# sencheng/CoBeL-RL

Measured on AMD Instinct MI355X. Metric: gridworld env-steps/sec (whole job), higher is better.
Workload: dtype f32

## Files before the change

cobel-rl_amd/csrc/tabular_pwg.hip:

```cpp
#include <stdlib.h>
#include <string.h>

#include "cobel_common.h"
#include "cobel_policy.h"

namespace {

constexpr int kHashBytes = 128 * 8;
constexpr int kMaxSlices = 8;
constexpr uint32_t kWholeTicket = 0x40000000u;
constexpr uint32_t kWholeThenSlices = 0x80000000u;
constexpr uint32_t kWholeSlice = 0xffu;
constexpr uint32_t kAbortWord = COBEL_TAB_SCRATCH_ABORT_WORD;
constexpr uint32_t kRingSpinLimit = 1u << 22;
struct pwg_args {
  const cobel_wrec* rec;
  const uint16_t* starts;
  const int32_t* start_off;
  int32_t S, n_worlds;
  cobel_tab_run_t r;
  uint64_t thr[16][3];
  float alpha_f, gamma_f, model_lr_f;
  int32_t nl, ng;
  uint32_t* queue;
  uint32_t reserve;
  int32_t n_slices;
  int32_t slice_steps[kMaxSlices];
  uint32_t whole;
  uint32_t* owner;
  uint32_t* tail;
  uint32_t* ring;
  uint32_t ring_stride;
  uint32_t xcc_limit;
};

#if defined(COBEL_PWG_NT)
#define NT_LD(p) __builtin_nontemporal_load(p)
#define NT_ST(v, p) __builtin_nontemporal_store(v, p)
#else
#define NT_LD(p) (*(p))
#define NT_ST(v, p) (*(p) = (v))
#endif

__device__ __forceinline__ void stores_done() { asm volatile("s_waitcnt vmcnt(0)" ::: "memory"); }

#if defined(COBEL_PWG_STAMPS)
__device__ __forceinline__ void pwg_stamp(uint32_t* stamps, uint32_t* prev, int k, int lane) {
  if (lane == 0) {
    const uint32_t now = (uint32_t)__builtin_readcyclecounter();
    atomicAdd(stamps + k, now - *prev);
    *prev = now;
  }
}
#define PWG_STAMP(k) pwg_stamp(stamps, stamp_prev, k, lane)
#else
#define PWG_STAMP(k)
#endif

typedef const __attribute__((address_space(4))) pwg_args* pwg_kargs;
__device__ __forceinline__ pwg_kargs rare_args() {
#if defined(__HIP_DEVICE_COMPILE__)
  pwg_kargs p = (pwg_kargs)__builtin_amdgcn_kernarg_segment_ptr();
  asm volatile("" : "+s"(p));
  return p;
#else
  return nullptr;
#endif
}

template <bool QG, bool POW2>
__device__ __forceinline__ void pwg_instance(const pwg_args& A, const int i, const int step_budget,
                                             unsigned char* const lds, const int lane,
                                             const uint64_t thr_mine, const uint32_t stripe
#if defined(COBEL_PWG_STAMPS)
                                             , uint32_t* stamps, uint32_t* stamp_prev
#endif
                                             ) {
  const int S = A.S;
  float4* const Qs = reinterpret_cast<float4*>(lds);
  float* const Qf = reinterpret_cast<float*>(lds);
  unsigned long long* const H = reinterpret_cast<unsigned long long*>(lds);
  const uint32_t g = A.r.instance_base + (uint32_t)i;
  const int world = (int)(g % (uint32_t)A.n_worlds);
  const uint4* const W4 = reinterpret_cast<const uint4*>(A.rec + (size_t)world * S);
  float4* const Qg = reinterpret_cast<float4*>(A.r.q) + (size_t)i * S;
  float* const Qgf = reinterpret_cast<float*>(Qg);
  uint64_t* const model = A.r.model + (size_t)i * S * 4;
  const uint32_t* const model32 = reinterpret_cast<const uint32_t*>(model);
  const uint32_t SA = (uint32_t)S * 4u;
  uint16_t* const Mg = A.r.model_index + (size_t)i * SA;
  uint32_t succ_sel = (lane & 2) ? 0xffffffffu : 0u, succ_sh = (uint32_t)(lane & 1) * 16u;
  uint32_t SAv = POW2 ? (uint32_t)__builtin_clz(SA) + 1u : SA;
  uint32_t qlane = (uint32_t)(lane & 3);
  asm volatile("" : "+v"(succ_sel), "+v"(succ_sh), "+v"(SAv), "+v"(qlane));
  auto succ_of = [&](uint32_t w0, uint32_t w1) -> uint32_t {
    return (((w1 & succ_sel) | (w0 & ~succ_sel)) >> succ_sh) & 0xffffu;
  };

  int32_t* const inst = A.r.inst + (size_t)i * COBEL_I_WORDS;
  int state = inst[COBEL_I_STATE];
  int step = inst[COBEL_I_STEP];
  int trial = inst[COBEL_I_TRIAL];
  uint32_t ce = (uint32_t)inst[COBEL_I_CTR_ENV];
  uint32_t cp = (uint32_t)inst[COBEL_I_CTR_POLICY];
  uint32_t cm = (uint32_t)inst[COBEL_I_CTR_MEMORY];
  uint32_t iflags = (uint32_t)inst[COBEL_I_FLAGS];
  double trew = *reinterpret_cast<const double*>(inst + COBEL_I_REWARD_LO + (lane & 0));
  asm volatile("" : "+v"(trew));
  uint32_t nonzero = 0u;
  if (QG) {
    for (int s0 = 0; s0 < S; s0 += 512) {
      float4 qv[8];
#pragma unroll
      for (int j = 0; j < 8; ++j) {
        const int s = s0 + j * 64 + lane;
        qv[j] = Qg[s < S ? s : S - 1];
      }
#pragma unroll
      for (int j = 0; j < 8; ++j)
        nonzero |= fbits(qv[j].x) | fbits(qv[j].y) | fbits(qv[j].z) | fbits(qv[j].w);
    }
  } else {
    for (int s0 = 0; s0 < S; s0 += 64) {
      const int s = s0 + lane;
      if (s < S)
        __builtin_amdgcn_global_load_lds(
            (const __attribute__((address_space(1))) void*)(Qg + s),
            (__attribute__((address_space(3))) void*)(Qs + s0), 16, 0, 0);
    }
  }

  const int B = A.r.batch;
#if defined(COBEL_PWG_SSEED)
  auto seed_now = [&]() -> uint64_t {
    uint64_t sd = A.r.seed;
    asm volatile("" : "+s"(sd));
    return sd;
  };
#else
  uint64_t seed_v = A.r.seed;
  asm volatile("" : "+v"(seed_v));
  auto seed_now = [&]() -> uint64_t { return seed_v; };
#endif
  double alpha = A.r.alpha, gamma = A.r.gamma;
  float alpha_f = A.alpha_f, gamma_f = A.gamma_f, mlr_f = A.model_lr_f;
  asm volatile("" : "+v"(alpha), "+v"(gamma), "+v"(alpha_f), "+v"(gamma_f), "+v"(mlr_f));

  uint32_t cw0 = 0, cw1 = 0;
  uint4 cand = {0, 0, 0, 0};
  cobel_u4 blk = {0, 0, 0, 0};
  int refresh_in = 0;
  uint2 mdig = {0u, 0u};
  uint32_t fix_sa = ~0u;
  float fix_r = 0.0f;
  uint32_t idx_cur = 0, mg_cur = 0;

  auto draw_m = [&](uint32_t counter) -> uint32_t {
    const cobel_u4 b = cobel_philox(counter >> 2, (uint32_t)lane, g, COBEL_STREAM_MEMORY, seed_now());
    return cobel_word(b, counter & 3u);
  };
  auto refresh_draws = [&](uint32_t pq) {
    const uint32_t mi = (cm + 1u) >> 2;
    const bool p0 = lane == 62, p1 = lane == 63;
    blk = cobel_philox(p1 ? 2u * pq + 1u : (p0 ? 2u * pq : mi), (p0 || p1) ? 0u : (uint32_t)lane,
                       g, (p0 || p1) ? COBEL_STREAM_POLICY : COBEL_STREAM_MEMORY, seed_now());
  };
  auto enter_state = [&](int s) {
    const uint4 c = W4[s];
    cw0 = rfl(c.x);
    cw1 = rfl(c.y);
    cand = W4[succ_of(cw0, cw1)];
    mdig = *reinterpret_cast<const uint2*>(&Mg[(uint32_t)s * 4u]);
  };
  auto begin_trial = [&]() -> bool {
    const pwg_kargs R = rare_args();
    if (trial >= R->r.trials_target) return false;
    const int start_lo = R->start_off[world];
    const uint32_t start_cnt = (uint32_t)(R->start_off[world + 1] - start_lo);
    state = (int)R->starts[start_lo + (int)cobel_draw_bounded(ce, 0u, g, COBEL_STREAM_ENV, seed_now(),
                                                              start_cnt)];
    ce += 1u;
    step = 0;
    trew = 0.0;
    asm volatile("" : "+v"(trew));
    iflags |= 1u;
    enter_state(state);
    return true;
  };
  auto plan_td = [&](float q, float m, float r, uint32_t nt) -> float {
    const double gnt = gamma * (double)nt;
    double td = (double)r + gnt * (double)m;
    td = td - (double)q;
    return (float)((double)q + alpha * td);
  };
  auto conflict_sets = [&](uint32_t idx, uint32_t ns) -> unsigned long long {
    unsigned long long* const H1 = H;
    unsigned long long* const H2 = H + 64;
    const uint32_t h1 = idx & 63u, h2 = idx >> 6;
    const unsigned long long bit = 1ull << lane;
    atomicOr(&H1[h1], bit);
    atomicOr(&H2[h2], bit);
    __builtin_amdgcn_wave_barrier();
    const ulonglong2* const r4 = reinterpret_cast<const ulonglong2*>(&H1[(ns & 15u) * 4u]);
    const ulonglong2 ra = r4[0], rb = r4[1];
    const unsigned long long cell = H1[h1] & H2[h2];
    const unsigned long long row = ((ra.x | ra.y) | (rb.x | rb.y)) & H2[ns >> 4];
    const unsigned long long cnd = (cell | row) & (bit - 1ull);
    __builtin_amdgcn_wave_barrier();
    H1[h1] = 0ull;
    H2[h2] = 0ull;
    return cnd;
  };
  uint32_t* const Qu = reinterpret_cast<uint32_t*>(lds);
  const uint4* const Qs4u = reinterpret_cast<const uint4*>(lds);
  uint32_t tag_mine = ~(uint32_t)lane;
  auto tag_round = [&](uint32_t idx, uint32_t ns, bool act, bool ch, float q, float qn, int lo) -> int {
    if (ch) atomicMax(&Qu[idx], tag_mine);
    __builtin_amdgcn_wave_barrier();
    uint32_t t = 0u, c2 = 0u;
    if (act) {
      const uint4 r2 = Qs4u[ns];
      c2 = Qu[idx];
      t = max(max(max(r2.x, r2.y), r2.z), max(r2.w, c2));
    }
    const unsigned long long blocked = __builtin_amdgcn_ballot_w64(act && t > tag_mine);
    const int stop = max(blocked ? __ffsll((long long)blocked) - 1 : B, lo + 1);
    if (ch && c2 == tag_mine) Qf[idx] = lane < stop ? qn : q;
    __builtin_amdgcn_wave_barrier();
    return stop;
  };
  auto run_batch_lds = [&](uint32_t idx, uint32_t ns, uint32_t nt, float r) {
    int first;
    {
      const float4 row = Qs[ns];
      const float q = Qf[idx];
      const float qn = plan_td(q, max4(row), r, nt);
      const bool ch = fbits(qn) != fbits(q);
      if (!__builtin_amdgcn_ballot_w64(ch)) return;
      first = tag_round(idx, ns, true, ch, q, qn, 0);
    }
    while (first < B) {
      const bool act = lane >= first;
      float q = 0.0f, qn = 0.0f;
      if (act) {
        const float4 row = Qs[ns];
        q = Qf[idx];
        qn = plan_td(q, max4(row), r, nt);
      }
      const bool ch = act && fbits(qn) != fbits(q);
      if (!__ballot(ch)) return;
      first = tag_round(idx, ns, act, ch, q, qn, first);
    }
  };
  auto run_batch_glb = [&](uint32_t idx, uint32_t ns, uint32_t nt, float r, float4 row, float q) {
    int first = B;
    bool have_conf = false;
    unsigned long long conf = 0ull;
    auto take_writes = [&](unsigned long long pend, float qn) {
      while (__ballot(pend != 0ull)) {
        const int e = pend ? (__ffsll((long long)pend) - 1) : 0;
        const uint32_t ie = (uint32_t)__shfl((int)idx, e);
        const float ve = __shfl(qn, e);
        if (pend) {
          if (ie == idx) q = ve;
          if ((ie >> 2) == ns) {
            const uint32_t c = ie & 3u;
            row.x = c == 0u ? ve : row.x;
            row.y = c == 1u ? ve : row.y;
            row.z = c == 2u ? ve : row.z;
            row.w = c == 3u ? ve : row.w;
          }
          pend &= pend - 1ull;
        }
      }
    };
    {
      const float qn = plan_td(q, max4(row), r, nt);
      const bool ch = fbits(qn) != fbits(q);
      const unsigned long long changed = __builtin_amdgcn_ballot_w64(ch);
      if (!changed) return;
      conf = conflict_sets(idx, ns);
      have_conf = true;
      const unsigned long long blocked = __builtin_amdgcn_ballot_w64((conf & changed) != 0ull);
      if (blocked) first = __ffsll((long long)blocked) - 1;
      if (ch && lane < first) Qgf[idx] = qn;
      if (first < B) {
        const unsigned long long committed = changed & ((1ull << first) - 1ull);
        take_writes(lane >= first ? (conf & committed) : 0ull, qn);
      }
    }
    while (first < B) {
      const bool act = lane >= first;
      float qn = q;
      if (act) qn = plan_td(q, max4(row), r, nt);
      const bool ch = act && fbits(qn) != fbits(q);
      const unsigned long long changed = __ballot(ch);
      int stop = B;
      if (changed) {
        if (!have_conf) {
          conf = conflict_sets(idx, ns);
          have_conf = true;
        }
        const unsigned long long blocked = __ballot(act && (conf & changed) != 0ull);
        if (blocked) stop = __ffsll((long long)blocked) - 1;
        if (ch && lane < stop) Qgf[idx] = qn;
        if (stop < B) {
          const unsigned long long committed = changed & ((1ull << stop) - 1ull);
          take_writes(lane >= stop ? (conf & committed) : 0ull, qn);
        }
      }
      first = stop;
    }
  };

  uint32_t warm;
  {
    const uint32_t off = (uint32_t)lane * 128u, last = SA * 2u - 4u;
    warm = *reinterpret_cast<const uint32_t*>(reinterpret_cast<const char*>(Mg) + (off < last ? off : last));
  }
  bool live = true;
  if (iflags & 1u) enter_state(state);
  else live = begin_trial();
  refresh_draws(cp >> 2);
  {
    const int jp = 3 - (int)(cp & 3u), jm = 4 - (int)((cm + 1u) & 3u);
    refresh_in = jp < jm ? jp : jm;
  }
  idx_cur = lane < B ? cobel_bounded(draw_m(cm), SA) : 0u;
  mg_cur = lane < B ? (uint32_t)Mg[idx_cur] : 0u;
  asm volatile("" ::"v"(warm));
  if (!QG) {
    stores_done();
    for (int s = lane; s < S; s += 64) {
      const float4 qv = Qs[s];
      nonzero |= fbits(qv.x) | fbits(qv.y) | fbits(qv.z) | fbits(qv.w);
    }
  }
  if (QG) {
    for (int b = lane; b < 128; b += 64) H[b] = 0ull;
    __builtin_amdgcn_wave_barrier();
  }
  if (!__ballot(nonzero != 0u)) {
    const uint2* const M2 = reinterpret_cast<const uint2*>(Mg);
    for (int s0 = 0; s0 < S; s0 += 512) {
      uint2 mv[8];
#pragma unroll
      for (int j = 0; j < 8; ++j) {
        const int s = s0 + j * 64 + lane;
        mv[j] = M2[s < S ? s : S - 1];
      }
#pragma unroll
      for (int j = 0; j < 8; ++j) nonzero |= (mv[j].x | mv[j].y) & 0x80008000u;
    }
  }
  if (__ballot(nonzero != 0u)) iflags |= 2u;

  PWG_STAMP(1);
  const int budget0 = step_budget > 0 ? step_budget : 0x7fffffff;
  int budget = budget0;
  uint32_t batches = 0u;
  asm volatile("" : "+v"(batches));

  while (live) {
    if (budget == 0) break;
    budget -= 1;

    const int src_lane = 62 + (int)((cp >> 1) & 1u);
    const uint32_t w0 = rl((cp & 1u) ? blk.z : blk.x, src_lane);
    const uint32_t w1 = rl((cp & 1u) ? blk.w : blk.y, src_lane);
    if (__builtin_expect(refresh_in == 0, 0)) {
      refresh_draws((cp + 1u) >> 2);
      const int jp = 4 - (int)((cp + 1u) & 3u), jm = 4 - (int)((cm + 1u) & 3u);
      refresh_in = jp < jm ? jp : jm;
    }
    refresh_in -= 1;
    cp += 1u;

    const uint32_t succ = succ_of(cw0, cw1);
    float4 srow;
    float qc;
    float4 prow = {0.0f, 0.0f, 0.0f, 0.0f};
    float pq = 0.0f;
    if (QG) {
      stores_done();
      qc = Qgf[(uint32_t)state * 4u + qlane];
      srow = Qg[succ];
      if (lane < B && (iflags & 2u)) {
        prow = Qg[mg_cur & 0x3fffu];
        pq = Qgf[idx_cur];
      }
    } else {
      qc = Qf[(uint32_t)state * 4u + qlane];
      srow = Qs[succ];
    }
    const float smax = max4(srow);

    int a;
    {
      float m;
      asm("s_nop 1\n\t"
          "v_max_f32_dpp %0, %1, %1 quad_perm:[1,0,3,2] row_mask:0xf bank_mask:0xf\n\t"
          "s_nop 1\n\t"
          "v_max_f32_dpp %0, %0, %0 quad_perm:[2,3,0,1] row_mask:0xf bank_mask:0xf"
          : "=&v"(m)
          : "v"(qc));
      const int t = (int)((uint32_t)__ballot(qc == m) & 15u);
      const uint64_t K = cobel_u53(w0, w1);
      const unsigned long long passed = __ballot(thr_mine <= K);
      a = __popcll((passed >> (t * 3)) & 7ull);
    }
    const int ns = (int)next_of(cw0, cw1, a);
    const uint32_t nw0 = rl(cand.x, a), nw1 = rl(cand.y, a);
    const uint32_t r_bits = rl(cand.z, a);
    const float r = __builtin_bit_cast(float, r_bits);
    if (r_bits != 0u) iflags |= 2u;
    const uint32_t end = rl(cand.w, a);
    const float ns_max = __builtin_bit_cast(float, rl(fbits(smax), a));
    const uint32_t nt = 1u - end;
    const uint32_t sa = (uint32_t)state * 4u + (uint32_t)a;
    const bool trial_over = end || (step + 1 >= A.r.steps_per_trial);
    const uint32_t dpair = rfl((a & 2) ? mdig.y : mdig.x);
    const uint32_t dold = (a & 1) ? (dpair >> 16) : (dpair & 0xffffu);
    float R = 0.0f;
    if (__builtin_expect((dold & 0x8000u) != 0u, 0)) {
      R = __builtin_bit_cast(float, rfl(model32[2u * sa]));
    }
    __builtin_amdgcn_sched_barrier(0);
    cand = W4[succ_of(nw0, nw1)];
    const uint2 mdig_next = *reinterpret_cast<const uint2*>(&Mg[(uint32_t)ns * 4u]);

    if (sa == fix_sa) R = fix_r;
    const float d = r - R;
    const float Rn = R + mlr_f * d;
    const uint32_t fresh_idx = sa;
    const float fresh_r = Rn;
    const uint32_t fresh_m = (uint32_t)ns | (nt << 14) | (fbits(Rn) ? 0x8000u : 0u);
    fix_sa = sa;
    fix_r = Rn;
    const float q_sa = __builtin_bit_cast(float, rl(fbits(qc), a));
    const float gnt = nt ? gamma_f : 0.0f;
    float td = r + gnt * ns_max;
    td = td - q_sa;
    const float qn_online = q_sa + alpha_f * td;
    if (lane == 0) {
      if (QG) Qgf[sa] = qn_online;
      else Qf[sa] = qn_online;
      NT_ST(cobel_model_pack(fresh_r, (uint32_t)ns, nt), &model[sa]);
      Mg[sa] = (uint16_t)fresh_m;
    }
    __builtin_amdgcn_wave_barrier();

    trew += (double)r;
    const int s_prev = state;
    state = ns;
    cw0 = nw0;
    cw1 = nw1;

    {
      uint32_t idx_next = 0u, mg_next = 0u;
      const uint32_t m = (idx_cur == fresh_idx) ? fresh_m : mg_cur;
      if (lane < B) {
        float rj = 0.0f;
        idx_next = POW2 ? cobel_word(blk, (cm + 1u) & 3u) >> SAv
                        : cobel_bounded(cobel_word(blk, (cm + 1u) & 3u), SAv);
        mg_next = (uint32_t)Mg[idx_next];
        if (iflags & 2u) {
          batches += 1u;
          if (__builtin_expect((m & 0x8000u) != 0u, 0)) {
            rj = __builtin_bit_cast(float, model32[2u * idx_cur]);
            asm volatile("" : "+v"(rj));
          }
          if (idx_cur == fresh_idx) rj = fresh_r;
          const uint32_t nsj = m & 0x3fffu;
          if (QG) {
            if (__ballot(idx_cur == fresh_idx)) {
              const float4 nrow = {__builtin_bit_cast(float, rl(fbits(srow.x), a)),
                                   __builtin_bit_cast(float, rl(fbits(srow.y), a)),
                                   __builtin_bit_cast(float, rl(fbits(srow.z), a)),
                                   __builtin_bit_cast(float, rl(fbits(srow.w), a))};
              if (idx_cur == fresh_idx) prow = nrow;
            }
            if (idx_cur == sa) pq = qn_online;
            if (nsj == (uint32_t)s_prev) {
              prow.x = a == 0 ? qn_online : prow.x;
              prow.y = a == 1 ? qn_online : prow.y;
              prow.z = a == 2 ? qn_online : prow.z;
              prow.w = a == 3 ? qn_online : prow.w;
            }
            run_batch_glb(idx_cur, nsj, (m >> 14) & 1u, rj, prow, pq);
          } else {
            run_batch_lds(idx_cur, nsj, (m >> 14) & 1u, rj);
          }
        }
        if (idx_next == fresh_idx) mg_next = fresh_m;
      }
      idx_cur = idx_next;
      mg_cur = mg_next;
      mdig = mdig_next;
      cm += 1u;
    }

    if (__builtin_expect(trial_over, 0)) {
      const pwg_kargs R = rare_args();
#define rr (R->r)
      if (lane == 0 && trial >= 0 && trial < rr.trial_cap) {
        const size_t mo = (size_t)stripe * (size_t)rr.trial_cap + (size_t)trial;
        if (rr.lat_sum) atomicAdd(rr.lat_sum + mo, (unsigned long long)step);
        if (rr.lat_cnt) atomicAdd(rr.lat_cnt + mo, 1ull);
        if (rr.reward_sum) atomicAdd(rr.reward_sum + mo, trew);
        if (rr.resp_cnt && trew > 0.0) atomicAdd(rr.resp_cnt + mo, 1ull);
        if (rr.lat_trace) rr.lat_trace[(size_t)i * rr.trial_cap + trial] = step;
      }
#undef rr
      trial += 1;
      iflags &= ~1u;
      if (!begin_trial()) break;
    } else {
      step += 1;
    }
  }

  __builtin_amdgcn_wave_barrier();
  PWG_STAMP(2);
  if (!QG) {
    for (int s0 = 0; s0 < S; s0 += 256) {
      float4 qv[4];
#pragma unroll
      for (int j = 0; j < 4; ++j) {
        const int s = s0 + j * 64 + lane;
        qv[j] = Qs[s < S ? s : S - 1];
      }
#pragma unroll
      for (int j = 0; j < 4; ++j) {
        const int s = s0 + j * 64 + lane;
        if (s < S) Qg[s] = qv[j];
      }
    }
  }
  if (lane == 0) {
    inst[COBEL_I_STATE] = state;
    inst[COBEL_I_STEP] = step;
    inst[COBEL_I_TRIAL] = trial;
    inst[COBEL_I_CTR_ENV] = (int32_t)ce;
    inst[COBEL_I_CTR_POLICY] = (int32_t)cp;
    inst[COBEL_I_CTR_MEMORY] = (int32_t)cm;
    inst[COBEL_I_FLAGS] = (int32_t)(iflags & ~2u);
    const unsigned long long executed = (unsigned long long)(budget0 - budget);
    *reinterpret_cast<double*>(inst + COBEL_I_REWARD_LO) = trew;
    *reinterpret_cast<unsigned long long*>(inst + COBEL_I_STEPS_LO) += executed;
    const pwg_kargs R = rare_args();
    if (R->r.steps_done && executed) atomicAdd(R->r.steps_done, executed);
    if (R->r.batches_done && batches) atomicAdd(R->r.batches_done, (unsigned long long)batches);
  }
  __builtin_amdgcn_wave_barrier();
}

template <bool SLICED, bool POW2>
__global__ __launch_bounds__(1024) void k_tab_pwg(const pwg_args A) {
  extern __shared__ __attribute__((aligned(16))) unsigned char lds_raw[];
  const int lane = (int)(threadIdx.x & 63u);
  const int wave = (int)rfl(threadIdx.x >> 6);
  const int waves = A.nl + A.ng;
  const size_t slice_l = (size_t)A.S * 16;
  const bool qg = wave >= A.nl;
  unsigned char* const lds =
      lds_raw + (qg ? (size_t)A.nl * slice_l + (size_t)(wave - A.nl) * kHashBytes
                    : (size_t)wave * slice_l);
  const uint64_t thr_mine = A.thr[(lane % 48) / 3][lane % 3];
  const uint32_t wave_id = (uint32_t)blockIdx.x * (uint32_t)waves + (uint32_t)wave;
  const uint32_t stripe = A.r.mon_stripes > 1 ? wave_id % (uint32_t)A.r.mon_stripes : 0u;
#if defined(COBEL_PWG_STAMPS)
  uint32_t* const stamps = A.ring + (size_t)8 * A.ring_stride + (size_t)wave_id * 8u;
  uint32_t* const stamp_prev = reinterpret_cast<uint32_t*>(
      lds_raw + (size_t)A.nl * slice_l + (size_t)A.ng * kHashBytes + (size_t)wave * 8);
  if (lane == 0) {
    *stamp_prev = (uint32_t)__builtin_readcyclecounter();
    stamps[7] = (uint32_t)__builtin_amdgcn_s_memrealtime();
  }
#endif
  uint32_t xcc;
  asm volatile("s_getreg_b32 %0, hwreg(HW_REG_XCC_ID)" : "=s"(xcc));
  xcc &= 7u;
  if (SLICED && xcc > A.xcc_limit) return;
  uint32_t tstate = xcc << 8;
  uint32_t t_next = 0xffffffffu;
  for (;;) {
    int i = -1;
    {
      constexpr bool sliced = SLICED;
      uint32_t k0 = tstate & 0xffu;
      const uint32_t x = (tstate >> 8) & 0xffu;
      uint32_t sl = 0u;
      while (k0 < 8u) {
        const uint32_t q = (x + k0) & 7u;
        const uint32_t nq = ((uint32_t)A.r.n + 7u - q) / 8u;
        const uint32_t nw = sliced ? min(nq, A.whole & 0xffffffu) : 0u;
        const uint32_t ns = nq - nw;
        const uint32_t total = SLICED ? ns * (uint32_t)A.n_slices : ns;
        uint32_t t = t_next;
        t_next = 0xffffffffu;
        if (t >= total) t = 0xffffffffu;
        if (t == 0xffffffffu) {
          t = 0x10000000u;
          if (lane == 0 && nq) {
            bool serve = true;
            if (sliced) {
              uint32_t o = __hip_atomic_load(A.owner + q, __ATOMIC_RELAXED, __HIP_MEMORY_SCOPE_AGENT);
              if (o == 0u) {
                o = atomicCAS(A.owner + q, 0u, x + 1u);
                if (o == 0u) o = x + 1u;
              }
              serve = o == x + 1u;
            }
            if (serve) {
              if (qg && nw) {
                const uint32_t b = atomicAdd(A.queue + q * 8u + 1u, 1u);
                if (b < nw) t = kWholeTicket | b;
              }
              if (t == 0x10000000u && !(qg && nw && !(A.whole & kWholeThenSlices)) &&
                  !(qg && __hip_atomic_load(A.queue + q * 8u, __ATOMIC_RELAXED,
                                            __HIP_MEMORY_SCOPE_AGENT) + A.reserve >= total)) {
                t = atomicAdd(A.queue + q * 8u, 1u);
                if (t >= total) {
                  t = 0x10000000u;
                  if (nw) {
                    const uint32_t b = atomicAdd(A.queue + q * 8u + 1u, 1u);
                    if (b < nw) t = kWholeTicket | b;
                  }
                }
              }
            }
          }
          t = rfl(t);
        }
        if (SLICED && (t & kWholeTicket)) {
          i = (int)((t & 0xffffffu) * 8u + q);
          sl = kWholeSlice;
          break;
        }
        if (t < total) {
          if (t < ns) {
            i = (int)((nw + t) * 8u + q);
          } else {
            const uint32_t* const slot = A.ring + (size_t)q * A.ring_stride + (t - ns);
            uint32_t e, spins = 0u;
            while ((e = rfl(__hip_atomic_load(slot, __ATOMIC_RELAXED, __HIP_MEMORY_SCOPE_AGENT))) == 0u) {
              __builtin_amdgcn_s_sleep(32);
              ++spins;
              if (spins >= kRingSpinLimit ||
                  ((spins & 1023u) == 0u &&
                   rfl(__hip_atomic_load(A.queue + kAbortWord, __ATOMIC_RELAXED,
                                         __HIP_MEMORY_SCOPE_AGENT)) != 0u)) {
                if (lane == 0)
                  __hip_atomic_store(A.queue + kAbortWord, 1u, __ATOMIC_RELAXED,
                                     __HIP_MEMORY_SCOPE_AGENT);
                return;
              }
            }
            __builtin_amdgcn_fence(__ATOMIC_ACQUIRE, "agent");
            sl = e >> 24;
            i = (int)(((e & 0xffffffu) - 1u) * 8u + q);
          }
          break;
        }
        k0 += 1u;
      }
      tstate = k0 | (x << 8) | (sl << 16);
    }
#if defined(COBEL_PWG_STAMPS)
    if (i < 0 && lane == 0) {
      stamps[5] = tstate >> 8 & 0xffu;
      stamps[6] = (uint32_t)__builtin_amdgcn_s_memrealtime();
    }
#endif
    if (i < 0) break;
    int budget = A.r.step_budget;
    if (SLICED) {
      const int slice = (int)(tstate >> 16);
#pragma unroll
      for (int j = 0; j < kMaxSlices; ++j)
        if (j == slice) budget = A.slice_steps[j];
    }
#if defined(COBEL_PWG_STAMPS)
    PWG_STAMP(0);
    if (lane == 0) atomicAdd(stamps + 4, 1u);
    if (qg) pwg_instance<true, POW2>(A, i, budget, lds, lane, thr_mine, stripe, stamps, stamp_prev);
    else pwg_instance<false, POW2>(A, i, budget, lds, lane, thr_mine, stripe, stamps, stamp_prev);
    PWG_STAMP(3);
#else
    if (qg) pwg_instance<true, POW2>(A, i, budget, lds, lane, thr_mine, stripe);
    else pwg_instance<false, POW2>(A, i, budget, lds, lane, thr_mine, stripe);
#endif
    if (SLICED) {
      const uint32_t q = (uint32_t)i & 7u;
      const uint32_t sl1 = (tstate >> 16) + 1u;
      const bool more = sl1 < (uint32_t)A.n_slices;
      uint32_t pos = 0u, t = 0xffffffffu;
      if (lane == 0) {
        if (more) pos = atomicAdd(A.tail + q * 8u, 1u);
        if (!qg) t = atomicAdd(A.queue + q * 8u, 1u);
      }
      __builtin_amdgcn_fence(__ATOMIC_RELEASE, "workgroup");
      stores_done();
      if (lane == 0 && more)
        __hip_atomic_store(A.ring + (size_t)q * A.ring_stride + pos,
                           (((uint32_t)i >> 3) + 1u) | (sl1 << 24), __ATOMIC_RELAXED,
                           __HIP_MEMORY_SCOPE_AGENT);
      t_next = rfl(t);
    }
  }
}

}

bool cobel_tab_pwg_plan(const cobel_world* world, const cobel_tab_run_t& r, int* nl_out, int* ng_out,
                        size_t* lds_out) {
  static const char* const force = cobel_debug_env("COBEL_DEBUG_PWG");
  const int S = world->n_states;
  if (r.agent != COBEL_AGENT_DYNAQ || !r.model_index || r.occupancy || r.param_index ||
      r.last_exp || S * 4 > 4096 || S <= 256 || r.batch < 1 || r.batch > COBEL_MAX_BATCH)
    return false;
  const bool scratch = r.scratch && r.scratch_bytes >= COBEL_TAB_SCRATCH_BYTES(r.n);
  if (!scratch && !world->queue) return false;
  int n_cu = 0;
  size_t total = 0;
  if (cobel_device_limits(world->device, &n_cu, &total) != COBEL_OK) return false;
  const size_t slice_l = (size_t)S * 16;
#if defined(COBEL_PWG_STAMPS)
  total -= 1024;
#endif
  int nl = (int)(total / slice_l);
  if (nl > 16) nl = 16;
  int ng = 0;
  if (force) {
    int a = 0, b = 0;
    if (sscanf(force, "%d,%d", &a, &b) == 2 && a >= 0 && b >= 0 && a + b >= 1 && a + b <= 16 &&
        (size_t)a * slice_l + (size_t)b * kHashBytes <= total) {
      nl = a;
      ng = b;
    }
  } else if (r.flags & COBEL_F_PWG_GLOBAL) {
    nl = 0;
    ng = 16;
  } else if (128 / ((slice_l + 1279) / 1280) >= 16) {
    return false;
  }
  *nl_out = nl;
  *ng_out = ng;
  *lds_out = (size_t)nl * slice_l + (size_t)ng * kHashBytes;
  return true;
}

static int plan_slices(const cobel_tab_run_t& r, int grid, int n_cu, int nl, int ng, bool scratch,
                       int32_t* steps , uint32_t* whole) {
  const char* const forced = cobel_debug_env("COBEL_DEBUG_PWG_SLICES");
  for (int j = 0; j < kMaxSlices; ++j) steps[j] = 0;
  steps[0] = r.step_budget;
  *whole = 0u;
  if (!scratch || grid < n_cu || r.step_budget < 64) return 1;
  if (forced) {
    int v[kMaxSlices] = {0}, k = 0, sum = 0;
    const char* c = forced;
    while (k < kMaxSlices && *c) {
      v[k] = atoi(c);
      if (v[k] <= 0) break;
      sum += v[k++];
      while (*c && *c != ',') ++c;
      if (*c == ',') ++c;
    }
    if (k >= 1 && sum == r.step_budget) {
      for (int j = 0; j < k; ++j) steps[j] = v[j];
      return k;
    }
    return 1;
  }
  const double rounds = (double)r.n / ((double)grid * (nl + ng));
  const int b = r.step_budget;
  if (rounds < 1.0) return 1;
  if (ng == 0) {
    if (rounds >= 10.0) return 1;
    steps[1] = rounds >= 5.0 ? b / 8 : b / 4;
    steps[0] = b - steps[1];
    return 2;
  }
  if (rounds >= 14.0) return 1;
  if (rounds >= 7.0) {
    steps[1] = b / 8;
    steps[0] = b - steps[1];
    return 2;
  }
  if (rounds >= 3.5) {
    if (rounds >= 4.5 && nl > 0)
      *whole = (uint32_t)(2 * ((ng * grid + 7) / 8)) | kWholeThenSlices;
    steps[1] = b / 4;
    steps[0] = b - steps[1];
    return 2;
  }
  if (rounds >= 1.75 && nl > 0) {
    *whole = (uint32_t)((ng * grid + 7) / 8);
    steps[1] = b / 4;
    steps[0] = b - steps[1];
    return 2;
  }
  steps[2] = b / 8;
  steps[1] = b / 4;
  steps[0] = b - steps[1] - steps[2];
  return 3;
}

int cobel_tab_pwg_launch(const cobel_world* world, const cobel_tab_run_t& r, hipStream_t st) {
  int nl = 0, ng = 0;
  size_t lds = 0;
  if (!cobel_tab_pwg_plan(world, r, &nl, &ng, &lds))
    return cobel_fail(COBEL_E_UNSUPPORTED, "cobel_tab_pwg_launch: run not covered");
  pwg_args A;
  A.rec = world->rec;
  A.starts = world->starts;
  A.start_off = world->start_off;
  A.S = world->n_states;
  A.n_worlds = world->n_worlds;
  A.r = r;
  const cobel_eps_consts eps = cobel_make_eps_consts(r.epsilon);
  memcpy(A.thr, eps.thr, sizeof(A.thr));
  A.alpha_f = (float)r.alpha;
  A.gamma_f = (float)r.gamma;
  A.model_lr_f = (float)r.model_lr;
  A.nl = nl;
  A.ng = ng;
  int n_cu = 0;
  size_t lds_cu = 0;
  if (cobel_device_limits(world->device, &n_cu, &lds_cu) != COBEL_OK) return COBEL_E_HIP;
  const int waves = nl + ng;
  int grid = (r.n + waves - 1) / waves;
  if (grid > n_cu) grid = n_cu;
  const bool scratch = r.scratch && r.scratch_bytes >= COBEL_TAB_SCRATCH_BYTES(r.n);
  uint32_t* const base = scratch ? static_cast<uint32_t*>(r.scratch) : world->queue;
  A.queue = base;
  A.owner = scratch ? base + 64 : base;
  A.tail = scratch ? base + 128 : base;
  A.ring = scratch ? base + 256 : base;
  A.n_slices = plan_slices(r, grid, n_cu, nl, ng, scratch, A.slice_steps, &A.whole);
  A.ring_stride = (uint32_t)((r.n + 7) / 8) * (uint32_t)(A.n_slices - 1);
  {
    const char* const w_env = cobel_debug_env("COBEL_DEBUG_PWG_WHOLE");
    if (w_env) A.whole = (uint32_t)strtoul(w_env, nullptr, 0);
    if (nl == 0 || A.n_slices < 2) A.whole = 0u;
  }
  {
    const char* const m_env = cobel_debug_env("COBEL_DEBUG_PWG_XCCLIMIT");
    A.xcc_limit = m_env ? (uint32_t)atoi(m_env) & 7u : 7u;
  }
  {
    static const char* const k_env = cobel_debug_env("COBEL_DEBUG_PWG_RESERVE");
    const double k = k_env ? atof(k_env) : 2.0;
    A.reserve = nl ? (uint32_t)((double)nl * grid * k / 8.0) : 0u;
  }
#if defined(COBEL_PWG_STAMPS)
  lds += 1024;
  COBEL_HIP_TRY(hipMemsetAsync(base, 0, (256 + (size_t)8 * A.ring_stride + (size_t)8 * grid * waves) * 4, st));
#else
  COBEL_HIP_TRY(hipMemsetAsync(base, 0, scratch ? (size_t)kAbortWord * 4 : (size_t)256, st));
  if (A.n_slices > 1)
    COBEL_HIP_TRY(hipMemsetAsync(A.ring, 0, (size_t)8 * A.ring_stride * 4, st));
#endif
  const bool pow2 = (A.S & (A.S - 1)) == 0;
  void (*const kernel)(const pwg_args) =
      A.n_slices > 1 ? (pow2 ? &k_tab_pwg<true, true> : &k_tab_pwg<true, false>)
                     : (pow2 ? &k_tab_pwg<false, true> : &k_tab_pwg<false, false>);
  if (lds > 64 * 1024)
    COBEL_HIP_TRY(hipFuncSetAttribute(reinterpret_cast<const void*>(kernel),
                                      hipFuncAttributeMaxDynamicSharedMemorySize, (int)lds));
  hipLaunchKernelGGL(kernel, dim3(grid), dim3(64 * waves), lds, st, A);
  COBEL_HIP_TRY(hipGetLastError());
  return COBEL_OK;
}
```

Measured before the change: 3.093 billion.

## Add split head/tail instance scheduling for LDS-only pwg launches

```diff
diff --git a/cobel-rl_amd/csrc/tabular_pwg.hip b/cobel-rl_amd/csrc/tabular_pwg.hip
--- a/cobel-rl_amd/csrc/tabular_pwg.hip
+++ b/cobel-rl_amd/csrc/tabular_pwg.hip
@@ -11,6 +11,9 @@
 constexpr uint32_t kWholeTicket = 0x40000000u;
 constexpr uint32_t kWholeThenSlices = 0x80000000u;
 constexpr uint32_t kWholeSlice = 0xffu;
+constexpr uint32_t kNoTicket = 0x10000000u;
+constexpr uint32_t kHeadTicket = 0x20000000u;
+constexpr uint32_t kTailTicket = 0x40000000u;
 constexpr uint32_t kAbortWord = COBEL_TAB_SCRATCH_ABORT_WORD;
 constexpr uint32_t kRingSpinLimit = 1u << 22;
 struct pwg_args {
@@ -32,6 +35,9 @@
   uint32_t* ring;
   uint32_t ring_stride;
   uint32_t xcc_limit;
+  uint32_t split;
+  int32_t head_lo;
+  uint64_t head_step;
 };
 
 #if defined(COBEL_PWG_NT)
@@ -555,14 +561,14 @@
   __builtin_amdgcn_wave_barrier();
 }
 
-template <bool SLICED, bool POW2>
+template <bool SLICED, bool POW2, bool MIXED, bool SPLIT = false>
 __global__ __launch_bounds__(1024) void k_tab_pwg(const pwg_args A) {
   extern __shared__ __attribute__((aligned(16))) unsigned char lds_raw[];
   const int lane = (int)(threadIdx.x & 63u);
   const int wave = (int)rfl(threadIdx.x >> 6);
-  const int waves = A.nl + A.ng;
+  const int waves = MIXED ? A.nl + A.ng : A.nl;
   const size_t slice_l = (size_t)A.S * 16;
-  const bool qg = wave >= A.nl;
+  const bool qg = MIXED && wave >= A.nl;
   unsigned char* const lds =
       lds_raw + (qg ? (size_t)A.nl * slice_l + (size_t)(wave - A.nl) * kHashBytes
                     : (size_t)wave * slice_l);
@@ -572,7 +578,7 @@
 #if defined(COBEL_PWG_STAMPS)
   uint32_t* const stamps = A.ring + (size_t)8 * A.ring_stride + (size_t)wave_id * 8u;
   uint32_t* const stamp_prev = reinterpret_cast<uint32_t*>(
-      lds_raw + (size_t)A.nl * slice_l + (size_t)A.ng * kHashBytes + (size_t)wave * 8);
+      lds_raw + (size_t)A.nl * slice_l + (MIXED ? (size_t)A.ng * kHashBytes : 0) + (size_t)wave * 8);
   if (lane == 0) {
     *stamp_prev = (uint32_t)__builtin_readcyclecounter();
     stamps[7] = (uint32_t)__builtin_amdgcn_s_memrealtime();
@@ -581,12 +587,90 @@
   uint32_t xcc;
   asm volatile("s_getreg_b32 %0, hwreg(HW_REG_XCC_ID)" : "=s"(xcc));
   xcc &= 7u;
-  if (SLICED && xcc > A.xcc_limit) return;
+  static_assert(!SPLIT || (!SLICED && !MIXED), "split launches: whole tickets, LDS waves");
+  if ((SLICED || SPLIT) && xcc > A.xcc_limit) return;
   uint32_t tstate = xcc << 8;
   uint32_t t_next = 0xffffffffu;
   for (;;) {
     int i = -1;
-    {
+    int budget = A.r.step_budget;
+    if constexpr (SPLIT) {
+      uint32_t k0 = tstate & 0xffu;
+      const uint32_t x = (tstate >> 8) & 0xffu;
+      uint32_t kind = 0u;
+      while (k0 < 8u) {
+        const uint32_t q = (x + k0) & 7u;
+        const uint32_t nq = ((uint32_t)A.r.n + 7u - q) / 8u;
+        const uint32_t nsp = min(nq, A.split);
+        const uint32_t nwh = nq - nsp;
+        uint32_t t = kNoTicket, tt = t_next;
+        if (lane == 0 && nq) {
+          bool serve = false;
+          if (nsp) {
+            uint32_t o = __hip_atomic_load(A.owner + q, __ATOMIC_RELAXED, __HIP_MEMORY_SCOPE_AGENT);
+            if (o == 0u) {
+              o = atomicCAS(A.owner + q, 0u, x + 1u);
+              if (o == 0u) o = x + 1u;
+            }
+            serve = o == x + 1u;
+          }
+          if (serve && tt == 0xffffffffu &&
+              __hip_atomic_load(A.queue + q * 8u, __ATOMIC_RELAXED, __HIP_MEMORY_SCOPE_AGENT) < nsp) {
+            const uint32_t h = atomicAdd(A.queue + q * 8u, 1u);
+            if (h < nsp) t = kHeadTicket | h;
+            else if (h < 2u * nsp) tt = h;
+          }
+          if (t == kNoTicket && nwh) {
+            const uint32_t b = atomicAdd(A.queue + q * 8u + 1u, 1u);
+            if (b < nwh) t = nsp + b;
+          }
+          if (t == kNoTicket && serve) {
+            if (tt == 0xffffffffu) {
+              const uint32_t h = atomicAdd(A.queue + q * 8u, 1u);
+              if (h < 2u * nsp) tt = h;
+            }
+            if (tt != 0xffffffffu) {
+              t = kTailTicket | (tt - nsp);
+              tt = 0xffffffffu;
+            }
+          }
+        }
+        t = rfl(t);
+        t_next = rfl(tt);
+        if (t != kNoTicket) {
+          if (t & kTailTicket) {
+            const uint32_t* const slot = A.ring + (size_t)q * A.ring_stride + (t & 0xffffffu);
+            uint32_t e, spins = 0u;
+            while ((e = rfl(__hip_atomic_load(slot, __ATOMIC_RELAXED, __HIP_MEMORY_SCOPE_AGENT))) == 0u) {
+              __builtin_amdgcn_s_sleep(32);
+              ++spins;
+              if (spins >= kRingSpinLimit ||
+                  ((spins & 1023u) == 0u &&
+                   rfl(__hip_atomic_load(A.queue + kAbortWord, __ATOMIC_RELAXED,
+                                         __HIP_MEMORY_SCOPE_AGENT)) != 0u)) {
+                if (lane == 0)
+                  __hip_atomic_store(A.queue + kAbortWord, 1u, __ATOMIC_RELAXED,
+                                     __HIP_MEMORY_SCOPE_AGENT);
+                return;
+              }
+            }
+            __builtin_amdgcn_fence(__ATOMIC_ACQUIRE, "agent");
+            i = (int)((e - 1u) * 8u + q);
+            kind = 2u;
+          } else {
+            i = (int)((t & 0xffffffu) * 8u + q);
+            kind = (t & kHeadTicket) ? 1u : 0u;
+          }
+          break;
+        }
+        k0 += 1u;
+      }
+      tstate = k0 | (x << 8) | (kind << 16);
+      if (kind) {
+        const int head = A.head_lo + (int)(((uint64_t)(uint32_t)i * A.head_step) >> 16);
+        budget = kind == 1u ? head : budget - head;
+      }
+    } else {
       constexpr bool sliced = SLICED;
       uint32_t k0 = tstate & 0xffu;
       const uint32_t x = (tstate >> 8) & 0xffu;
@@ -594,7 +678,7 @@
       while (k0 < 8u) {
         const uint32_t q = (x + k0) & 7u;
         const uint32_t nq = ((uint32_t)A.r.n + 7u - q) / 8u;
-        const uint32_t nw = sliced ? min(nq, A.whole & 0xffffffu) : 0u;
+        const uint32_t nw = (MIXED && sliced) ? min(nq, A.whole & 0xffffffu) : 0u;
         const uint32_t ns = nq - nw;
         const uint32_t total = SLICED ? ns * (uint32_t)A.n_slices : ns;
         uint32_t t = t_next;
@@ -617,8 +701,8 @@
                 const uint32_t b = atomicAdd(A.queue + q * 8u + 1u, 1u);
                 if (b < nw) t = kWholeTicket | b;
               }
-              if (t == 0x10000000u && !(qg && nw && !(A.whole & kWholeThenSlices)) &&
-                  !(qg && __hip_atomic_load(A.queue + q * 8u, __ATOMIC_RELAXED,
+              if (t == 0x10000000u && !(MIXED && qg && nw && !(A.whole & kWholeThenSlices)) &&
+                  !(MIXED && qg && __hip_atomic_load(A.queue + q * 8u, __ATOMIC_RELAXED,
                                             __HIP_MEMORY_SCOPE_AGENT) + A.reserve >= total)) {
                 t = atomicAdd(A.queue + q * 8u, 1u);
                 if (t >= total) {
@@ -633,7 +717,7 @@
           }
           t = rfl(t);
         }
-        if (SLICED && (t & kWholeTicket)) {
+        if (MIXED && SLICED && (t & kWholeTicket)) {
           i = (int)((t & 0xffffffu) * 8u + q);
           sl = kWholeSlice;
           break;
@@ -674,7 +758,6 @@
     }
 #endif
     if (i < 0) break;
-    int budget = A.r.step_budget;
     if (SLICED) {
       const int slice = (int)(tstate >> 16);
 #pragma unroll
@@ -684,11 +767,11 @@
 #if defined(COBEL_PWG_STAMPS)
     PWG_STAMP(0);
     if (lane == 0) atomicAdd(stamps + 4, 1u);
-    if (qg) pwg_instance<true, POW2>(A, i, budget, lds, lane, thr_mine, stripe, stamps, stamp_prev);
+    if (MIXED && qg) pwg_instance<true, POW2>(A, i, budget, lds, lane, thr_mine, stripe, stamps, stamp_prev);
     else pwg_instance<false, POW2>(A, i, budget, lds, lane, thr_mine, stripe, stamps, stamp_prev);
     PWG_STAMP(3);
 #else
-    if (qg) pwg_instance<true, POW2>(A, i, budget, lds, lane, thr_mine, stripe);
+    if (MIXED && qg) pwg_instance<true, POW2>(A, i, budget, lds, lane, thr_mine, stripe);
     else pwg_instance<false, POW2>(A, i, budget, lds, lane, thr_mine, stripe);
 #endif
     if (SLICED) {
@@ -707,6 +790,16 @@
                            (((uint32_t)i >> 3) + 1u) | (sl1 << 24), __ATOMIC_RELAXED,
                            __HIP_MEMORY_SCOPE_AGENT);
       t_next = rfl(t);
+    }
+    if (SPLIT && ((tstate >> 16) & 0xffu) == 1u) {
+      const uint32_t q = (uint32_t)i & 7u;
+      uint32_t pos = 0u;
+      if (lane == 0) pos = atomicAdd(A.tail + q * 8u, 1u);
+      __builtin_amdgcn_fence(__ATOMIC_RELEASE, "workgroup");
+      stores_done();
+      if (lane == 0)
+        __hip_atomic_store(A.ring + (size_t)q * A.ring_stride + pos, ((uint32_t)i >> 3) + 1u,
+                           __ATOMIC_RELAXED, __HIP_MEMORY_SCOPE_AGENT);
     }
   }
 }
@@ -806,6 +899,36 @@
   steps[1] = b / 4;
   steps[0] = b - steps[1] - steps[2];
   return 3;
+}
+
+static uint32_t plan_split(const cobel_tab_run_t& r, int grid, int n_cu, int waves, bool scratch,
+                           int32_t* head_lo, uint64_t* head_step) {
+  const char* const forced = cobel_debug_env("COBEL_DEBUG_PWG_SPLIT");
+  const int b = r.step_budget;
+  const uint32_t per_queue = (uint32_t)((r.n + 7) / 8);
+  int lo = b / 32 < 8 ? 8 : b / 32, hi = b - lo;
+  uint32_t split = 0u;
+  *head_lo = 0;
+  *head_step = 0u;
+  if (!scratch || b < 64) return 0u;
+  if (forced) {
+    int k = 0, flo = lo, fhi = hi;
+    const int got = sscanf(forced, "%d,%d,%d", &k, &flo, &fhi);
+    if (got < 1 || k < 0 || (got == 3 && !(flo >= 1 && fhi > flo && fhi <= b))) return 0u;
+    if (got == 3) {
+      lo = flo;
+      hi = fhi;
+    }
+    split = (uint32_t)k;
+  } else {
+    if (grid < n_cu || (double)r.n / ((double)grid * waves) < 10.0) return 0u;
+    split = (uint32_t)((grid * waves + 7) / 8);
+  }
+  if (split > per_queue) split = per_queue;
+  if (split == 0u) return 0u;
+  *head_lo = lo;
+  *head_step = ((uint64_t)(hi - lo) << 16) / ((uint64_t)8 * split);
+  return split;
 }
 
 int cobel_tab_pwg_launch(const cobel_world* world, const cobel_tab_run_t& r, hipStream_t st) {
@@ -855,18 +978,29 @@
     const double k = k_env ? atof(k_env) : 2.0;
     A.reserve = nl ? (uint32_t)((double)nl * grid * k / 8.0) : 0u;
   }
+  const bool mixed = ng > 0 || A.whole != 0u;
+  A.split = 0u;
+  A.head_lo = 0;
+  A.head_step = 0u;
+  if (!mixed && A.n_slices == 1) {
+    A.split = plan_split(r, grid, n_cu, waves, scratch, &A.head_lo, &A.head_step);
+    if (A.split) A.ring_stride = A.split;
+  }
 #if defined(COBEL_PWG_STAMPS)
   lds += 1024;
   COBEL_HIP_TRY(hipMemsetAsync(base, 0, (256 + (size_t)8 * A.ring_stride + (size_t)8 * grid * waves) * 4, st));
 #else
   COBEL_HIP_TRY(hipMemsetAsync(base, 0, scratch ? (size_t)kAbortWord * 4 : (size_t)256, st));
-  if (A.n_slices > 1)
+  if (A.n_slices > 1 || A.split)
     COBEL_HIP_TRY(hipMemsetAsync(A.ring, 0, (size_t)8 * A.ring_stride * 4, st));
 #endif
   const bool pow2 = (A.S & (A.S - 1)) == 0;
   void (*const kernel)(const pwg_args) =
-      A.n_slices > 1 ? (pow2 ? &k_tab_pwg<true, true> : &k_tab_pwg<true, false>)
-                     : (pow2 ? &k_tab_pwg<false, true> : &k_tab_pwg<false, false>);
+      A.split ? (pow2 ? &k_tab_pwg<false, true, false, true> : &k_tab_pwg<false, false, false, true>) :
+      mixed ? (A.n_slices > 1 ? (pow2 ? &k_tab_pwg<true, true, true> : &k_tab_pwg<true, false, true>)
+                              : (pow2 ? &k_tab_pwg<false, true, true> : &k_tab_pwg<false, false, true>))
+            : (A.n_slices > 1 ? (pow2 ? &k_tab_pwg<true, true, false> : &k_tab_pwg<true, false, false>)
+                              : (pow2 ? &k_tab_pwg<false, true, false> : &k_tab_pwg<false, false, false>));
   if (lds > 64 * 1024)
     COBEL_HIP_TRY(hipFuncSetAttribute(reinterpret_cast<const void*>(kernel),
                                       hipFuncAttributeMaxDynamicSharedMemorySize, (int)lds));
```

New measurement: 3.054 billion. 0.987x the previous value.
